# mxy-kit/poisson-ellipse-openmp-mpi-cuda

Hardware: AMD Instinct MI355X
Metric: pcg_iters_per_sec_8192x8192 (higher is better)
Workload: dtype fp64

## Files before the change

csrc/hip/fused3.hip:

```cpp
#include <cstdlib>

#include "peer_sum.hpp"
#include "sstep.hpp"

#pragma clang fp contract(fast)

namespace pe {
namespace dev {

namespace {

constexpr int H3 = 6;
constexpr int FSW3 = kFSW3;
constexpr int HL3 = kHL3, HR3 = 64 - kFSW3 - kHL3;
static_assert(HL3 >= H3 && HR3 >= H3, "three-step strip: 64 loaded columns (one per lane), >= H3 halo lanes per side");
#ifndef PE_S3_XD
#define PE_S3_XD 3
#endif
#ifndef PE_S3_WD
#define PE_S3_WD 3
#endif
#ifndef PE_S3_NTX
#define PE_S3_NTX 0
#endif
constexpr int kS3XD = PE_S3_XD, kS3WD = PE_S3_WD;
static_assert(6 % kS3XD == 0 && 6 % kS3WD == 0, "register ring periods must divide the 6-step group");
constexpr int NS = kNS3;
constexpr int kRing3 = 7;
using WaveTV3 = WaveTV1<kRing3>;

struct Coef3 {
  double zc[3], a[3], b[3], cw[3];
};

struct Scal3 {
  bool first;
  long long K;
  int m;
  int brk;
  bool bad;
  Coef3 c;
  double g[3];
};

__device__ __forceinline__ double mform(const double (&xz)[3], const double (&xp)[3], const double (&mzz)[6],
                                        const double (&mzp)[6], const double (&mpp)[6], int sh) {
  double s = 0.0;
#pragma unroll
  for (int a = 0; a < 3; ++a)
#pragma unroll
    for (int b = 0; b < 3; ++b) {
      const int n = a + b + sh;
      s += xz[a] * (xz[b] * mzz[n] + 2.0 * xp[b] * mzp[n]) + xp[a] * xp[b] * mpp[n];
    }
  return s;
}

struct St3 {
  long long iter, brk3, k0;
  int done, late3, wpar, started, bad3;
  double gprev;
  double n2[2][3];
  double sc[12];
  double R[16];
};
__device__ __forceinline__ St3 st3_load(const DevState* st, int par) {
  St3 S;
  S.done = st->done;
  S.iter = st->iter;
  S.late3 = st->late3;
  S.wpar = st->wpar;
  S.started = st->started;
  S.bad3 = st->bad3;
  S.brk3 = st->brk3;
  S.k0 = st->k0;
  S.gprev = st->gprev;
#pragma unroll
  for (int i = 0; i < 3; ++i) {
    S.n2[0][i] = st->fs2[0][16 + i];
    S.n2[1][i] = st->fs2[1][16 + i];
  }
#pragma unroll
  for (int i = 0; i < 12; ++i) S.sc[i] = st->sc3[i];
  const double* R = st->fs2[par ^ 1];
#pragma unroll
  for (int i = 0; i < 16; ++i) S.R[i] = R[i];
  return S;
}

__device__ __forceinline__ Scal3 sweep3_scalars(const KParams& k, const St3& st, int par) {
  Scal3 c;
  c.first = st.started == 0;
  c.K = st.iter;
  c.m = 0;
  c.brk = 0;
  c.bad = false;
#pragma unroll
  for (int i = 0; i < 3; ++i) {
    c.c.zc[i] = 0.0;
    c.c.a[i] = 0.0;
    c.c.b[i] = 1.0;
    c.c.cw[i] = 0.0;
    c.g[i] = 0.0;
  }
  if (c.first) return c;
  const double hh = k.h1 * k.h2;
// ... 119 lines not shown
  p.n = m0;
#pragma unroll
  for (int i = 0; i < 3; ++i)
    if (i < m0) {
      p.d[i] = late_diff(k, st, i);
      p.a[i] = st.sc[3 + i];
      p.b[i] = st.sc[6 + i];
      p.g[i] = st.sc[9 + i];
    }
}
__device__ __forceinline__ void pend3_record(const KParams& k, DevState* st, const Pend3& p) {
#pragma unroll
  for (int i = 0; i < 3; ++i)
    if (i < p.n) {
      hist_put(k, p.K0 + i + 1, p.d[i]);
      if (i + 1 == p.n) {
        st->last_diff = p.d[i];
        st->alpha = p.a[i];
        st->beta = p.b[i];
        st->rz_cur = p.g[i];
      }
    }
}

__device__ __forceinline__ void sweep3_finalize(const KParams& k, DevState* st, int par, const Scal3& c,
                                                const double (&t)[NS], const Pend3& pend) {
  if (!c.first) pend3_record(k, st, pend);
#pragma unroll
  for (int n = 0; n < NS; ++n) st->fs2[par][n] = t[n];
  if (!c.first && k.fault_iter > c.K && k.fault_iter <= c.K + c.m) st->fs2[par][1] = __builtin_nan("");
  if (!c.first && k.fault_zero > c.K && k.fault_zero <= c.K + c.m)
    st->fs2[par][1] = st->fs2[par][6] = st->fs2[par][11] = 0.0;
  st->wpend = 0;
  st->wpar = par;
  if (c.first) {
    st->started = 1;
    return;
  }
#pragma unroll
  for (int i = 0; i < 3; ++i) {
    st->sc3[i] = c.c.zc[i];
    st->sc3[3 + i] = c.c.a[i];
    st->sc3[6 + i] = c.c.b[i];
    st->sc3[9 + i] = c.g[i];
    if (i + 1 == c.m) {
      st->alpha = c.c.a[i];
      st->beta = c.c.b[i];
      st->rz_cur = c.g[i];
      st->gprev = c.g[i];
    }
  }
  st->iter = c.K + c.m;
  st->late3 = c.m;
  st->brk3 = c.brk ? c.K + c.brk : 0;
  st->bad3 = c.bad ? 1 : 0;
}

enum { kMixed = 0, kBand = 1, kUniform = 2 };

struct M3Ctx {
  const double* Xm;
  double* Ym;
  double* Wm;
  const double* hrd;
  int64_t pitch, poff, wp;
  int J, c0, ib, ie, t0, tmax, nx, par;
  unsigned off;
  bool lv0, o0, fix;
  bool scol;
  double lf0;
  double ih1, ih2, dcl;
  int rlo, rhi;
  double zc1, zc2, zc3, a1, a2, a3, b1, b2, b3, w1, w2, w3;
};

struct M3Rings {
  double RQ[kS3XD], PQ[kS3XD], WQ[kS3WD];
  double P1[3], RI[2], R1[2], P2[3], R2[2], P3[3], Z[3], S[2], U[3], V[3], UU[3], VV[3];
  bool pushed;
};

typedef __attribute__((address_space(1))) char gchar3;
typedef __attribute__((address_space(1))) double gdouble3;
struct M3Ptr {
  const gchar3* xi;
  gchar3* yo;
  gchar3* wo;
  unsigned pb, wb;
  unsigned roff, poffb, wloff;
};

struct Pre3 {
  int2 e;
  int4 rc4;
  bool staged;
};

template <bool STEADY>
__device__ __forceinline__ URow urow(const M3Ctx& c, int q) {
  URow r{c.ih1, c.ih2, c.dcl};
  if constexpr (!STEADY) {
    if (!(q >= c.rlo && q <= c.rhi)) r.d = 0.0;
  }
  return r;
}

template <bool PUSH>
__device__ __forceinline__ double ldx3(const KParams& k, const M3Ctx& c, int t, unsigned o) {
  if constexpr (PUSH) {
    if ((t < 1 && k.has[LEFT]) || (t > c.nx && k.has[RIGHT])) {
      const double* h = c.hrd + int64_t(t < 1 ? t + H3 - 1 : t - c.nx + H3 - 1) * c.pitch + o;
      return __hip_atomic_load(h, __ATOMIC_RELAXED, __HIP_MEMORY_SCOPE_SYSTEM);
    }
  }
#if PE_S3_NTX
  return __builtin_nontemporal_load(c.Xm + int64_t(t) * c.pitch + o);
#else
  return c.Xm[int64_t(t) * c.pitch + o];
#endif
}

__device__ __forceinline__ double ldxb3(const gchar3* base, unsigned& off) {
  asm("" : "+v"(off));
#if PE_S3_NTX
  return __builtin_nontemporal_load(reinterpret_cast<const gdouble3*>(base + off));
#else
  return *reinterpret_cast<const gdouble3*>(base + off);
#endif
}
__device__ __forceinline__ double ldntb3(const gchar3* base, unsigned& off) {
  asm("" : "+v"(off));
  return __builtin_nontemporal_load(reinterpret_cast<const gdouble3*>(base + off));
}
__device__ __forceinline__ void stntb3(gchar3* base, unsigned& off, double v) {
  asm("" : "+v"(off));
  __builtin_nontemporal_store(v, reinterpret_cast<gdouble3*>(base + off));
}

__device__ __forceinline__ double ldnt1(const double* p) { return __builtin_nontemporal_load(p); }
__device__ __forceinline__ void stnt1(double* p, double v) { __builtin_nontemporal_store(v, p); }

__device__ __forceinline__ void push_row3(const KParams& k, const M3Ctx& c, M3Rings& x, int q, double r3, double p3) {
  auto put = [&](double* base, int slot) {
    double* d = base + int64_t(slot) * c.pitch + c.off;
    if (c.o0) {
      __hip_atomic_store(d, r3, __ATOMIC_RELAXED, __HIP_MEMORY_SCOPE_SYSTEM);
      __hip_atomic_store(d + c.poff, p3, __ATOMIC_RELAXED, __HIP_MEMORY_SCOPE_SYSTEM);
    }
    x.pushed = true;
  };
  if (q <= H3 && k.hpush_lo[c.par] != nullptr) put(k.hpush_lo[c.par], q - 1);
  if (q >= c.nx - H3 + 1 && k.hpush_hi[c.par] != nullptr) put(k.hpush_hi[c.par], q - (c.nx - H3 + 1));
}

template <int KIND, bool PUSH, bool EDGE, bool STEADY, int JJ>
__device__ __forceinline__ void step3(const KParams& k, const M3Ctx& c, M3Rings& x, M3Ptr& rp, const RowCtx& rx,
                                      WaveTV3& tvw, double (&sv)[NS], int n, int bs) {
  constexpr bool BAND = KIND == kBand, UNI = KIND == kUniform;
  constexpr int XD = kS3XD, WD = kS3WD;
  const double zc1 = c.zc1, zc2 = c.zc2, zc3 = c.zc3, w1 = c.w1, w2 = c.w2, w3 = c.w3;
  constexpr int m0 = JJ % 3, m1 = (JJ + 2) % 3, m2 = (JJ + 1) % 3;
  constexpr int e0 = JJ & 1, e1 = (JJ + 1) & 1;
  constexpr int xs = JJ % XD, ws = JJ % WD;
  const int t = c.t0 + n;
  const int c0 = c.c0;
  auto inr = [&](int q) { return STEADY ? !c.fix : (q >= c.ib && q <= c.ie); };
  auto own = [&](int q) { return STEADY || (q >= c.ib && q <= c.ie); };
  auto put = [&](int n, double v) {
    if constexpr (UNI) sv[n] += v;
    else sv[n] += c.scol ? v : 0.0;
  };
  auto interior = [&](int q) { return q >= c.rlo && q <= c.rhi; };
  auto live = [&](int d) { return STEADY || n >= 2 * d; };
  int bsl[7];
#pragma unroll
  for (int d = 0; d < 7; ++d) bsl[d] = bs >= d ? bs - d : bs - d + kRing3;
  auto zmask = [&](int q, double v, double d) -> double {
    if constexpr (UNI) {
      return EDGE ? (v * d) * c.lf0 : v * d;
    } else {
      return (interior(q) && c.lv0) ? v * d : 0.0;
    }
  };
  auto op = [&](int q, int sl, int sln, double um, double u0, double un, double& d) {
    if constexpr (UNI) {
      const URow r = urow<STEADY>(c, q);
      d = r.d;
      return lapu(r, um, u0, un);
    } else {
      return apply_row1<BAND>(k, rx, tvw, q, c0, sl, sln, um, u0, un, d);
    }
  };
  auto pnext = [&](double zc, double z, double b, double p, bool zfused) -> double {
    if constexpr (UNI) return zfused ? __builtin_fma(zc, z, b * p) : __builtin_fma(b, p, zc * z);
    else return zc * z + b * p;
  };
  constexpr bool kAzf = STEADY && (PUSH ? JJ >= 3 : (!EDGE && JJ >= 4));
  const double rin = x.RQ[xs], pin = x.PQ[xs], wrow = x.WQ[ws];
  if constexpr (STEADY) {
    const int tn = t + XD;
    if (PUSH && ((tn < 1 && k.has[LEFT]) || (tn > c.nx && k.has[RIGHT]))) {
      x.RQ[xs] = ldx3<PUSH>(k, c, tn, c.off);
      x.PQ[xs] = ldx3<PUSH>(k, c, tn, unsigned(c.poff) + c.off);
    } else {
      x.RQ[xs] = ldxb3(rp.xi, rp.roff);
      x.PQ[xs] = ldxb3(rp.xi, rp.poffb);
    }
    x.WQ[ws] = c.o0 ? ldntb3(rp.wo, rp.wloff) : 0.0;
  } else {
    const int tn = min(t + XD, c.tmax);
    x.RQ[xs] = ldx3<PUSH>(k, c, tn, c.off);
    x.PQ[xs] = ldx3<PUSH>(k, c, tn, unsigned(c.poff) + c.off);
    const int wr = min(max(t - 2 + WD, c.ib), c.ie);
    x.WQ[ws] = c.o0 ? ldnt1(c.Wm + int64_t(wr) * c.wp + c.off) : 0.0;
  }
  {
    double d;
    if constexpr (UNI) d = urow<STEADY>(c, t).d;
    else d = BAND ? enter_band1(k, rx, tvw, t, c0, bsl[0]) : dinv_plain1(k, rx, t, c0);
    const double z = zmask(t, rin, d);
    x.P1[m0] = pnext(zc1, z, c.b1, pin, kAzf);
    x.RI[e0] = rin;
  }
  if (STEADY) __builtin_amdgcn_sched_barrier(0);
  if (live(1)) {
    const int q = t - 1;
    double d;
    const double s1 = op(q, bsl[1], bsl[0], x.P1[m2], x.P1[m1], x.P1[m0], d);
    const double r1 = x.RI[e1] - c.a1 * s1;
    const double z = zmask(q, r1, d);
    const double p1 = x.P1[m1];
    x.R1[e1] = r1;
    x.P2[m1] = pnext(zc2, z, c.b2, p1, false);
    if (inr(q)) put(16, p1 * p1);
  }
  if (STEADY) __builtin_amdgcn_sched_barrier(0);
  if (live(2)) {
    const int q = t - 2;
    double d;
    const double s2 = op(q, bsl[2], bsl[1], x.P2[m0], x.P2[m2], x.P2[m1], d);
    const double r2 = x.R1[e0] - c.a2 * s2;
    const double z = zmask(q, r2, d);
    const double p2 = x.P2[m2];
    x.R2[e0] = r2;
    const double p3 = pnext(zc3, z, c.b3, p2, false);
    x.P3[m2] = p3;
    if (own(q) && c.o0) {
      const double wn = wrow + w1 * x.P1[m2] + w2 * p2 + w3 * p3;
      if constexpr (STEADY) stntb3(rp.wo, rp.roff, wn);
      else stnt1(c.Wm + int64_t(q) * c.wp + c.off, wn);
    }
    if (inr(q)) put(17, p2 * p2);
  }
  if (STEADY) __builtin_amdgcn_sched_barrier(0);
  if (live(3)) {
    const int q = t - 3;
    double d;
    const double s3 = op(q, bsl[3], bsl[2], x.P3[m1], x.P3[m0], x.P3[m2], d);
    const double r3 = x.R2[e1] - c.a3 * s3;
    const double z = zmask(q, r3, d);
    x.Z[m0] = z;
    x.S[e1] = s3;
    const double p3 = x.P3[m0];
    if (own(q) && !c.fix) {
      if (c.o0) {
        if constexpr (STEADY) {
          stntb3(rp.yo, rp.roff, r3);
          stntb3(rp.yo, rp.poffb, p3);
        } else {
          double* yr = c.Ym + int64_t(q) * c.pitch + c.off;
          stnt1(yr, r3);
          stnt1(yr + c.poff, p3);
        }
      }
      if constexpr (PUSH) push_row3(k, c, x, q, r3, p3);
    }
    if (inr(q)) {
      put(0, r3 * z);
      put(6, z * s3);
      put(11, p3 * s3);
      put(18, p3 * p3);
    }
  }
  if (STEADY) __builtin_amdgcn_sched_barrier(0);
  if (live(4)) {
    const int q = t - 4;
    double d;
    const double qv = op(q, bsl[4], bsl[3], x.Z[m2], x.Z[m1], x.Z[m0], d);
    const double sr = x.S[e0];
    const double u = zmask(q, qv, d);
    const double v = zmask(q, sr, d);
    x.U[m1] = u;
    x.V[m1] = v;
    if (inr(q)) {
      put(1, x.Z[m1] * qv);
      put(2, qv * u);
      put(7, qv * v);
      put(12, sr * v);
    }
  }
  if (STEADY) __builtin_amdgcn_sched_barrier(0);
  if (live(5)) {
    const int q = t - 5;
    double d, d2;
    const double au = op(q, bsl[5], bsl[4], x.U[m0], x.U[m2], x.U[m1], d);
    const double av = op(q, bsl[5], bsl[4], x.V[m0], x.V[m2], x.V[m1], d2);
    const double uu = zmask(q, au, d);
    const double vv = zmask(q, av, d);
    x.UU[m2] = uu;
    x.VV[m2] = vv;
    if (inr(q)) {
      const double u = x.U[m2], v = x.V[m2];
      put(3, u * au);
      put(8, u * av);
      put(13, v * av);
      put(4, au * uu);
      put(9, au * vv);
      put(14, av * vv);
    }
  }
  if (STEADY) __builtin_amdgcn_sched_barrier(0);
  {
    const int q = t - 6;
    if (inr(q)) {
      double d;
      const double auu = op(q, bsl[6], bsl[5], x.UU[m1], x.UU[m0], x.UU[m2], d);
      const double avv = op(q, bsl[6], bsl[5], x.VV[m1], x.VV[m0], x.VV[m2], d);
      const double uu = x.UU[m0], vv = x.VV[m0];
      put(5, uu * auu);
      put(10, uu * avv);
      put(15, vv * avv);
    }
  }
  if constexpr (STEADY) {
    rp.xi += rp.pb;
    rp.yo += rp.pb;
    rp.wo += rp.wb;
    asm("" : "+s"(rp.xi), "+s"(rp.yo), "+s"(rp.wo));
  }
}

template <int KIND, bool PUSH, bool EDGE, bool STEADY>
__device__ __forceinline__ void group3(const KParams& k, const M3Ctx& c, M3Rings& x, M3Ptr& rp, const RowCtx& rx,
                                       WaveTV3& tvw, double (&sv)[NS], int n0, int nsteps, int& bs) {
  auto adv = [&]() { bs = bs == kRing3 - 1 ? 0 : bs + 1; };
#define PE_STEP3(JJ)                                                              \
  if (STEADY || n0 + JJ < nsteps) {                                               \
    step3<KIND, PUSH, EDGE, STEADY, JJ>(k, c, x, rp, rx, tvw, sv, n0 + JJ, bs);   \
    adv();                                                                        \
    if (STEADY) __builtin_amdgcn_sched_barrier(0);                                \
  }
  PE_STEP3(0)
  PE_STEP3(1)
  PE_STEP3(2)
  PE_STEP3(3)
  PE_STEP3(4)
  PE_STEP3(5)
#undef PE_STEP3
}

__device__ __forceinline__ unsigned long long rtc3() {
  unsigned long long t;
  asm volatile("s_memrealtime %0\n\ts_waitcnt lgkmcnt(0)" : "=s"(t)::"memory");
  return t;
}

__device__ __forceinline__ void prio_turn(const KParams& k) {
  if (k.prio > 0) {
    const unsigned long long t = rtc3();
    const bool young = int(blockIdx.x) >= k.ncu;
    if ((((t >> k.prio) & 1ull) != 0) != young) __builtin_amdgcn_s_setprio(1);
    else __builtin_amdgcn_s_setprio(0);
  }
}

template <int KIND, bool PUSH, bool EDGE, bool SST = false>
__device__ __forceinline__ void march3(const KParams& k, const Coef3& cf, bool fix, int par, int s, int ib, int ie,
                                       WaveTV3& tvw, double (&sv)[NS], unsigned long long* sst, const Pre3& pre,
                                       bool use_pre) {
  const int lane = threadIdx.x & 63;
  const int ny = int(k.ny);
  M3Ctx c;
  c.pitch = k.pitch;
  c.poff = k.poff;
  c.wp = k.wpitch;
  c.Xm = k.x[par ^ 1] - (HL3 - 1);
  c.Ym = k.x[par] - (HL3 - 1);
  c.Wm = k.w - (HL3 - 1);
  c.J = -(HL3 - 1) + s * FSW3;
  c.c0 = c.J + lane;
  c.off = unsigned(c.c0 + HL3 - 1);
  const int64_t g0 = k.gj0 + c.c0;
  c.lv0 = c.c0 <= ny + H3 && g0 >= 1 && g0 <= k.N - 1;
  c.lf0 = c.lv0 ? 1.0 : 0.0;
  c.o0 = lane >= HL3 && lane < 64 - HR3 && c.c0 >= 1 && c.c0 <= ny;
  c.scol = c.c0 <= ny;
  c.fix = fix;
  c.ib = ib;
  c.ie = ie;
  c.t0 = ib - H3;
  c.tmax = ie + H3;
  c.nx = int(k.nx);
  c.par = par;
  c.hrd = PUSH ? k.hrecv + int64_t(par ^ 1) * 2 * H3 * k.pitch : nullptr;
  c.rlo = int(max<int64_t>(1 - k.gi0, -(1 << 30)));
  c.rhi = int(min<int64_t>(k.M - 1 - k.gi0, 1 << 30));
  c.zc1 = cf.zc[0];
  c.zc2 = cf.zc[1];
  c.zc3 = cf.zc[2];
  c.a1 = cf.a[0];
  c.a2 = cf.a[1];
  c.a3 = cf.a[2];
  c.b1 = cf.b[0];
  c.b2 = cf.b[1];
  c.b3 = cf.b[2];
  c.w1 = cf.cw[0];
  c.w2 = cf.cw[1];
  c.w3 = cf.cw[2];
  asm("" : "+v"(c.w1), "+v"(c.w2), "+v"(c.w3));

  RowCtx rx;
  auto load_seg = [&](int base) { load_rows<KIND == kBand, WaveTV3, 64>(k, rx, tvw, base, ie + H3 + 1, c.J); };
  if (KIND == kBand) load_strip_tables1(k, tvw, c.c0);
  if (use_pre) load_rows<KIND == kBand, WaveTV3, 64>(k, rx, tvw, c.t0, ie + H3 + 1, c.J, &pre.rc4);
  else load_seg(c.t0);
  if constexpr (KIND == kUniform) {
    const bool in = rx.allin & 1ull;
    c.ih1 = in ? k.ih1sq : uni(k.inv_eps * k.ih1sq);
    c.ih2 = in ? k.ih2sq : uni(k.inv_eps * k.ih2sq);
    c.dcl = in ? k.dinv_in : k.dinv_out;
  } else {
    c.ih1 = c.ih2 = c.dcl = 0.0;
  }

  M3Rings x;
  x.pushed = false;
  constexpr int XD = kS3XD, WD = kS3WD;
  static_assert(WD <= 6, "the first WD w rows are all row ib (t0 - 2 + q < ib)");
  if (use_pre && pre.staged && KIND != kBand) {
    asm volatile("s_waitcnt vmcnt(0)" ::: "memory");
    const double* L = &tvw.a0r[0][0];
#pragma unroll
    for (int q = 0; q < XD; ++q) {
      x.RQ[q] = L[q * 128 + lane];
      x.PQ[q] = L[q * 128 + 64 + lane];
    }
    const double w0 = L[XD * 128 + lane];
#pragma unroll
    for (int q = 0; q < WD; ++q) x.WQ[q] = c.o0 ? w0 : 0.0;
  } else {
#pragma unroll
    for (int q = 0; q < XD; ++q) {
      const int t = min(c.t0 + q, c.tmax);
      x.RQ[q] = ldx3<PUSH>(k, c, t, c.off);
      x.PQ[q] = ldx3<PUSH>(k, c, t, unsigned(c.poff) + c.off);
    }
#pragma unroll
    for (int q = 0; q < WD; ++q)
      x.WQ[q] = c.o0 ? ldnt1(c.Wm + int64_t(min(max(c.t0 - 2 + q, ib), ie)) * c.wp + c.off) : 0.0;
  }
#pragma unroll
  for (int q = 0; q < 3; ++q) x.P1[q] = x.P2[q] = x.P3[q] = x.Z[q] = x.U[q] = x.V[q] = x.UU[q] = x.VV[q] = 0.0;
#pragma unroll
  for (int q = 0; q < 2; ++q) x.RI[q] = x.R1[q] = x.R2[q] = x.S[q] = 0.0;

  const int nsteps = ie + H3 - c.t0 + 1;
  const int rows = ie - ib + 1;
  int bs = 0;
  int sg = 3;
  if constexpr (SST) {
    if (sst && lane == 0) sst[2] = rtc3();
  }
  auto sstamp = [&]() {
    if constexpr (SST) {
      if (sst && lane == 0 && sg < 28) sst[sg] = rtc3();
      ++sg;
    }
    prio_turn(k);
  };
  auto reload = [&](int n0) {
    if (KIND != kUniform && c.t0 + n0 + 6 - rx.segbase > 63) load_seg(c.t0 + n0 - H3);
  };
  M3Ptr rp;
  rp.pb = unsigned(c.pitch) * 8u;
  rp.wb = unsigned(c.wp) * 8u;
  rp.roff = c.off * 8u;
  rp.poffb = (unsigned(c.poff) + c.off) * 8u;
  rp.wloff = rp.roff + unsigned(WD) * rp.wb;
  rp.xi = nullptr;
  rp.yo = rp.wo = nullptr;
  int n0 = 0;
  const int nsteady_end = KIND == kUniform ? rows + 4 - 5 : -1;
  for (; n0 < nsteps && !(n0 >= 12 && n0 <= nsteady_end); n0 += 6) {
    reload(n0);
    group3<KIND, PUSH, EDGE, false>(k, c, x, rp, rx, tvw, sv, n0, nsteps, bs);
    sstamp();
  }
  if constexpr (KIND == kUniform) {
    rp.xi = (const gchar3*)(c.Xm + int64_t(c.t0 + n0 + XD) * c.pitch);
    rp.yo = (gchar3*)(c.Ym + int64_t(c.t0 + n0 - 3) * c.pitch);
    rp.wo = (gchar3*)(c.Wm + int64_t(c.t0 + n0 - 2) * c.wp);
    for (; n0 <= nsteady_end; n0 += 6) {
      reload(n0);
      group3<KIND, PUSH, EDGE, true>(k, c, x, rp, rx, tvw, sv, n0, nsteps, bs);
      sstamp();
    }
    for (; n0 < nsteps; n0 += 6) {
      reload(n0);
      group3<KIND, PUSH, EDGE, false>(k, c, x, rp, rx, tvw, sv, n0, nsteps, bs);
      sstamp();
    }
  }
  if constexpr (PUSH) {
    if (x.pushed) asm volatile("s_waitcnt vmcnt(0)" ::: "memory");
  }
}

__device__ __forceinline__ void pre_load3(const KParams& k, int gwave, Pre3& pr) {
  pr.e = make_int2(0, 0);
  if (!(gwave < k.lwaves && gwave < k.nslots)) return;
  pr.e = cload_i2(k.ilist + gwave);
  const int rows = pr.e.y >> 20;
  if (rows == 0) return;
  const int ib = pr.e.x & kRowMask3;
  const int ie = min(ib + rows - 1, int(k.nx));
  pr.rc4 = rowcls_entry(k, ib - H3, ie + H3 + 1);
}

template <bool PUSH>
__device__ __forceinline__ void stage_first3(const KParams& k, int par, WaveTV3& tv, Pre3& pr) {
  pr.staged = false;
  const int rows = pr.e.y >> 20;
  if (rows == 0 || !k.stage || (pr.e.x & kBandBit)) return;
  const int sx = pr.e.y & 0xFFFFF, ib = pr.e.x & kRowMask3;
  const int t0 = ib - H3;
  if (PUSH && (t0 < 1 || t0 + kS3XD - 1 > int(k.nx))) return;
  typedef __attribute__((address_space(3))) void* lds_ptr;
  typedef __attribute__((address_space(1))) const void* g_ptr;
  const int lane = threadIdx.x & 63;
  const double* Xm = k.x[par ^ 1] - (HL3 - 1) + sx * FSW3;
  const double* Wm = k.w - (HL3 - 1) + sx * FSW3;
  static_assert((kS3XD * 128 + 64) * sizeof(double) <= sizeof(tv.a0r) + sizeof(tv.b0r), "staged rows fit the face ring");
  double* L = &tv.a0r[0][0];
#pragma unroll
  for (int q = 0; q < kS3XD; ++q) {
    const char* rr = reinterpret_cast<const char*>(Xm + int64_t(t0 + q) * k.pitch);
    const char* pp = reinterpret_cast<const char*>(Xm + int64_t(t0 + q) * k.pitch + k.poff);
#pragma unroll
    for (int h = 0; h < 2; ++h) {
      __builtin_amdgcn_global_load_lds((g_ptr)(rr + 256 * h + 4 * lane), (lds_ptr)(L + q * 128 + 32 * h), 4, 0, 0);
      __builtin_amdgcn_global_load_lds((g_ptr)(pp + 256 * h + 4 * lane), (lds_ptr)(L + q * 128 + 64 + 32 * h), 4, 0, 0);
    }
  }
  const char* wr = reinterpret_cast<const char*>(Wm + int64_t(ib) * k.wpitch);
#pragma unroll
  for (int h = 0; h < 2; ++h)
    __builtin_amdgcn_global_load_lds((g_ptr)(wr + 256 * h + 4 * lane), (lds_ptr)(L + kS3XD * 128 + 32 * h), 4, 0, 0);
  pr.staged = true;
}

__device__ __forceinline__ Coef3 uni3(const Coef3& c) {
  Coef3 u;
#pragma unroll
  for (int i = 0; i < 3; ++i) {
    u.zc[i] = uni(c.zc[i]);
    u.a[i] = uni(c.a[i]);
    u.b[i] = uni(c.b[i]);
    u.cw[i] = uni(c.cw[i]);
  }
  return u;
}

enum { kPlain = 0, kStamp = 1, kReplay = 2, kSignal = 3 };

template <bool PUSH, int MODE>
__device__ __forceinline__ void walk3(const KParams& k, const Coef3& cf, bool fix, int par, WaveTV3& tv, int wid,
                                      double (&acc)[NS], const Pre3& pre, bool have_pre) {
  constexpr bool STAMP = MODE == kStamp;
  const int W = k.lwaves;
  const int gwave = int(blockIdx.x) * kWPB + wid;
  const bool l0 = (threadIdx.x & 63) == 0;
  if constexpr (STAMP) {
    if (l0) k.stamps[4 * int64_t(k.nslots) + 2 * gwave] = rtc3();
  }
  const int pend = gwave < W ? k.nslots : 0;
  unsigned long long* sst = STAMP ? k.stamps2 + 32 * int64_t(gwave) : nullptr;
  bool p1 = have_pre && !fix;
  bool ring_zeroed = false;
  for (int pos = gwave; pos < pend; pos += W) {
    const int2 e = p1 ? pre.e : cload_i2(k.ilist + pos);
    const int rows = e.y >> 20;
    if (rows == 0) {
      p1 = false;
      continue;
    }
    const int s = e.y & 0xFFFFF, ib = e.x & kRowMask3;
    const int ie = min(ib + rows - 1, int(k.nx));
    const unsigned long long t_item = STAMP ? rtc3() : 0ull;
    if constexpr (STAMP) {
      if (sst && l0) sst[0] = t_item;
    }
    if (e.x & kBandBit) {
      if (!ring_zeroed) {
        if (have_pre && pre.staged) asm volatile("s_waitcnt vmcnt(0)" ::: "memory");
        const int ln = threadIdx.x & 63;
        for (int i = ln; i < kRing3 * 64; i += 64) (&tv.a0r[0][0])[i] = 0.0;
        for (int i = ln; i < kRing3 * 66; i += 64) (&tv.b0r[0][0])[i] = 0.0;
        for (int i = ln; i < kRing3 * 64; i += 64) (&tv.d0r[0][0])[i] = 0.0;
        ring_zeroed = true;
      }
      march3<kBand, PUSH, true, STAMP>(k, cf, fix, par, s, ib, ie, tv, acc, sst, pre, p1);
    } else if (e.x & kUniBit) {
      const int c0 = -(HL3 - 1) + s * FSW3 + int(threadIdx.x & 63);
      const int64_t g0 = k.gj0 + c0;
      const bool lv = c0 <= int(k.ny) + H3 && g0 >= 1 && g0 <= k.N - 1;
      if (__ballot(lv) == ~0ull) march3<kUniform, PUSH, false, STAMP>(k, cf, fix, par, s, ib, ie, tv, acc, sst, pre, p1);
      else march3<kUniform, PUSH, true, STAMP>(k, cf, fix, par, s, ib, ie, tv, acc, sst, pre, p1);
    } else {
      march3<kMixed, PUSH, true, STAMP>(k, cf, fix, par, s, ib, ie, tv, acc, sst, pre, p1);
    }
    p1 = false;
    if constexpr (STAMP) {
      if (sst && l0) sst[31] = rtc3();
      sst = nullptr;
    }
    if constexpr (MODE == kSignal) {
      if (pos < k.lnb[0]) {
        asm volatile("s_waitcnt vmcnt(0)" ::: "memory");
        if (l0) __hip_atomic_fetch_add(&k.st->sig, 1ull, __ATOMIC_RELAXED, __HIP_MEMORY_SCOPE_AGENT);
      }
    }
    if constexpr (STAMP) {
      if (l0) {
        const unsigned long long kind = (e.x & kBandBit) ? 1ull : (e.x & kUniBit) ? 2ull : 0ull;
        unsigned long long* d = k.stamps + 4 * int64_t(pos);
        d[0] = t_item;
        d[1] = rtc3();
        d[2] = (unsigned long long)gwave | ((unsigned long long)s << 32);
        d[3] = (unsigned long long)ib | ((unsigned long long)(ie - ib + 1) << 32) | (kind << 48);
      }
    }
  }
  if constexpr (STAMP) {
    if (l0) {
      k.stamps[4 * int64_t(k.nslots) + 2 * gwave + 1] = rtc3();
      k.stamps2[32 * int64_t(gwave) + 29] = __builtin_amdgcn_s_memtime();
    }
  }
}

template <bool PUSH, int MODE = kPlain>
__global__ __launch_bounds__(TJ) __attribute__((amdgpu_waves_per_eu(2))) void kS3(KParams k, int par) {
  DevState* st = k.st;
  const St3 S = st3_load(st, par);
  const int done = S.done;
  __shared__ double sm[4 * NS];
  __shared__ int sflag;
  __shared__ WaveTV3 tvs[kWPB];
  __shared__ Pend3 pend;
  __shared__ Scal3 scl;
  const int lane = int(threadIdx.x & 63);
  const int wid = __builtin_amdgcn_readfirstlane(int(threadIdx.x >> 6));
  constexpr bool replay = MODE == kReplay;
  if constexpr (MODE == kStamp) {
    const unsigned long long t_in = rtc3();
    if (lane == 0) {
      k.stamps2[32 * (int64_t(blockIdx.x) * kWPB + wid) + 1] = t_in;
      const unsigned hw = __builtin_amdgcn_s_getreg(4 | (31 << 11)), xcc = __builtin_amdgcn_s_getreg(20 | (31 << 11));
      k.stamps2[32 * (int64_t(blockIdx.x) * kWPB + wid) + 30] = hw | (static_cast<unsigned long long>(xcc) << 32);
      k.stamps2[32 * (int64_t(blockIdx.x) * kWPB + wid) + 28] = __builtin_amdgcn_s_memtime();
      if (blockIdx.x == 0 && wid == 0) k.stamps2[-8] = k.stamps2[-6];
    }
  }
  if (done && !replay) return;
  Pre3 pre;
  const bool use_pre = !replay && k.pre_load;
  if (use_pre) {
    pre_load3(k, int(blockIdx.x) * kWPB + wid, pre);
    stage_first3<PUSH>(k, par, tvs[wid], pre);
  } else {
    pre.staged = false;
  }
  auto finish = [&](int upto, long long iter, int status, int fixj = 0) {
    if (arrive_last_wave(&st->ticket[4], gridDim.x * kWPB) && lane == 0) {
      sweep3_stop(k, st, upto, iter, status, fixj);
      __hip_atomic_store(&st->ticket[4], 0u, __ATOMIC_RELAXED, __HIP_MEMORY_SCOPE_AGENT);
    }
  };
  double acc[NS];
#pragma unroll
  for (int n = 0; n < NS; ++n) acc[n] = 0.0;
  const int m0 = S.late3;
  const long long K = S.iter, K0 = K - m0;
  auto pstamp = [&](int slot, double dep) {
// ... 145 lines not shown
```

csrc/hip/placement.cpp:

```cpp
#include <hip/hip_runtime_api.h>

#include <algorithm>
#include <chrono>
#include <cmath>
#include <cstdio>
#include <cstring>
#include <map>
#include <limits>
#include <mutex>
#include <queue>
#include <string>
#include <vector>

#include <rocprofiler-sdk-roctx/roctx.h>

#include "../hip/kernels.hpp"
#include "env_knobs.hpp"
#include "pe/device.hpp"
#include "solver_internal.hpp"

namespace pe {

namespace detail {
void* field_try_alloc(size_t bytes) {
  void* p = nullptr;
  if (hipMalloc(&p, bytes) != hipSuccess) {
    (void)hipGetLastError();
    return nullptr;
  }
  return p;
}

void* field_alloc(size_t bytes) {
  void* p = field_try_alloc(bytes);
  if (!p) PE_HIP_CHECK(hipErrorOutOfMemory);
  return p;
}

void field_free(void* p) {
  if (p) (void)hipFree(p);
}
}

using detail::clk;
using detail::field_free;
using detail::field_try_alloc;
using detail::Range;
using detail::secs;
using dev::KParams;

void DeviceSolver::choose_placement() {
  const double t_all = placement_s_;
  const auto t0 = clk::now();
  const bool fast = placement_search(false);
  if (comm_->size() > 1) {
    double v[1] = {(!placement_ms_.empty() && !fast) ? 1.0 : 0.0};
    comm_->host_max(v, 1, stream_);
    if (v[0] > 0.0 && !placement_ms_.empty() && !fast) placement_search(true);
    double m[1] = {placement_ms_.empty() ? 0.0 : double(placement_ms_[size_t(placement_best_)])};
    comm_->host_max(m, 1, stream_);
    placement_job_ms_ = m[0];
  } else if (!placement_ms_.empty()) {
    placement_job_ms_ = placement_ms_[size_t(placement_best_)];
  }
  placement_s_ = t_all + secs(t0, clk::now());
}

bool DeviceSolver::placement_search(bool retry) {
  Range range("pe.placement_search");
  double search_s = 0;
  struct Clock {
    double& out;
    clk::time_point t0 = clk::now();
    ~Clock() { out = secs(t0, clk::now()); }
  } clock{search_s};
  const double pts = double(blk_.nx) * double(blk_.ny);
  int tries = pts >= 24.0e6 ? 12 : 1;
  if (retry) tries = std::max(1, tries / 2 + 1);
  if (const std::optional<int> e = read_env_knobs().placement_tries) tries = std::max(1, *e);
  const double skip_gb = 8.0;
  const bool mid_large = pts < 50.0e6;
  const double fast_tbs = steps_ >= 3 ? (mid_large ? 4.0 : 4.6) : sstep_ ? 4.7 : 4.9, max_s = 0.3;
  if (tries <= 1) return true;
  {
    const double frac = 0.4;
    size_t free_b = 0, total_b = 0;
    if (hipMemGetInfo(&free_b, &total_b) == hipSuccess) {
      const double per_try = skip_gb * double(1ull << 30) + double(sizeof(double) * (2 * geo_.xsize + geo_.wsize));
      tries = std::min<int>(tries, std::max(1, int(frac * double(free_b) / per_try)));
    }
  }
  if (tries <= 1) return true;
  struct Cand {
    double *x0, *x1, *w;
    float ms;
  };
  std::vector<Cand> c;
  std::vector<void*> spacers;
  c.push_back(Cand{fields_, xalt_, walt_, 0.f});
  const size_t n_first = placement_ms_.size();
  if (retry && skip_gb > 0) {
    const double gb = double(n_first) * (skip_gb + double(sizeof(double) * (2 * geo_.xsize + geo_.wsize)) / double(1ull << 30));
    void* sp = nullptr;
    if (hipMalloc(&sp, size_t(gb * double(1ull << 30))) == hipSuccess) spacers.push_back(sp);
    else (void)hipGetLastError();
  }
  bool fast = false;
  for (int t = 0; t < tries; ++t) {
    if (t > 0) {
      void* sp = nullptr;
      if (skip_gb > 0 && hipMalloc(&sp, size_t(skip_gb * double(1ull << 30))) != hipSuccess) break;
      if (sp) spacers.push_back(sp);
      void* a = field_try_alloc(sizeof(double) * geo_.xsize);
      if (!a) break;
      void* b = field_try_alloc(sizeof(double) * geo_.xsize);
      if (!b) {
        field_free(a);
        break;
      }
      void* w = field_try_alloc(sizeof(double) * geo_.wsize);
      if (!w) {
        field_free(a);
        field_free(b);
        break;
      }
      c.push_back(Cand{static_cast<double*>(a), static_cast<double*>(b), static_cast<double*>(w), 0.f});
    }
    set_fused_fields(c[t].x0, c[t].x1, c[t].w);
    enqueue_init();
    dev::launch_S(*kp_, 1, stream_);
    for (int i = 0; i < 2; ++i) dev::launch_S(*kp_, i & 1, stream_);
    PE_HIP_CHECK(hipEventRecord(t0_, stream_));
    for (int i = 0; i < 6; ++i) dev::launch_S(*kp_, i & 1, stream_);
    PE_HIP_CHECK(hipEventRecord(t1_, stream_));
    PE_HIP_CHECK(hipEventSynchronize(t1_));
    PE_HIP_CHECK(hipEventElapsedTime(&c[t].ms, t0_, t1_));
    const double bps = sstep_ ? 48.0 : 40.0;
    const double tbs = bps * pts / (double(c[t].ms) / 6.0 * 1e-3) / 1e12;
    if (tbs >= fast_tbs) {
      fast = true;
      break;
    }
    if (secs(clock.t0, clk::now()) > max_s) break;
  }
  (void)hipGetLastError();
  size_t best = 0;
  for (size_t i = 1; i < c.size(); ++i)
    if (c[i].ms < c[best].ms) best = i;
  for (size_t i = 0; i < c.size(); ++i)
    if (i != best) {
      field_free(c[i].x0);
      field_free(c[i].x1);
      field_free(c[i].w);
    }
  for (void* sp : spacers) PE_HIP_CHECK(hipFree(sp));
  set_fused_fields(c[best].x0, c[best].x1, c[best].w);
  if (!retry) placement_ms_.clear();
  placement_best_ = int(placement_ms_.size() + best);
  for (const Cand& x : c) placement_ms_.push_back(x.ms / 6.0f);
  return fast || mid_large || (sstep_ ? 48.0 : 40.0) * pts / (double(c[best].ms) / 6.0 * 1e-3) / 1e12 >= fast_tbs;
}

}
```

csrc/hip/sstep.hpp:

```cpp
#pragma once

#include "kcommon.hpp"

#pragma clang fp contract(fast)

namespace pe {
namespace dev {
namespace {

__device__ __forceinline__ double2 dd(double a, double b) { return make_double2(a, b); }
__device__ __forceinline__ int2 cload_i2(const int2* p) {
  const long long v = cload(reinterpret_cast<const long long*>(p));
  return make_int2(int(v), int(v >> 32));
}

__device__ __forceinline__ double uni(double x) {
  const long long v = __double_as_longlong(x);
  const unsigned lo = unsigned(__builtin_amdgcn_readfirstlane(int(unsigned(v))));
  const unsigned hi = unsigned(__builtin_amdgcn_readfirstlane(int(v >> 32)));
  return __longlong_as_double((long long)((unsigned long long)hi << 32 | lo));
}

__device__ __forceinline__ double vreg(double x) {
  asm volatile("; vreg %0" : "+v"(x));
// ... 100 lines not shown
  double2 d, a0, b0;
  if (gen) {
    const int l = (q - rx.segbase) & 63;
    const int4 r4 = tv.rc[l];
    const RowCls rc{r4.x, r4.y, r4.z, r4.w};
    const CT ct{tv.half[l], tv.half[l + 1], tv.sB[l], tv.eB[l]};
    const CS x0 = cset_rc(k, rc, ct, c0, TV{tv.sA[jl], tv.eA[jl], tv.hB[jl], tv.hB[jl + 1]});
    const CS x1 = cset_rc(k, rc, ct, c0 + 1, TV{tv.sA[jl + 1], tv.eA[jl + 1], tv.hB[jl + 1], tv.hB[jl + 2]});
    d = dd(x0.d, x1.d);
    a0 = dd(x0.a0, x1.a0);
    b0 = dd(x0.b0, x1.b0);
  } else {
    const double f0 = in0 ? 1.0 : k.inv_eps, f1 = in1 ? 1.0 : k.inv_eps;
    d = dd(in0 ? k.dinv_in : k.dinv_out, in1 ? k.dinv_in : k.dinv_out);
    a0 = dd(f0, f1);
    b0 = a0;
  }
  *reinterpret_cast<double2*>(&tv.a0r[sl][jl]) = a0;
  *reinterpret_cast<double2*>(&tv.b0r[sl][jl]) = b0;
  __builtin_amdgcn_fence(__ATOMIC_RELEASE, "wavefront");
  __builtin_amdgcn_wave_barrier();
  __builtin_amdgcn_fence(__ATOMIC_ACQUIRE, "wavefront");
  return d;
}

template <bool BAND, class WT>
__device__ __forceinline__ double2 apply_row(const KParams& k, const RowCtx& rx, const WT& tv, int q, int c0, int jl,
                                             int sl, int sln, const double2& um, const double2& u0, const double2& un,
                                             double2& d) {
  const double ul = dpp_shr1(u0.y), ur = dpp_shl1(u0.x);
  bool in0, in1, gen;
  row_in(rx, q, c0, in0, in1, gen);
  if (BAND && gen) {
    const double2 a0 = *reinterpret_cast<const double2*>(&tv.a0r[sl][jl]);
    const double2 a1 = *reinterpret_cast<const double2*>(&tv.a0r[sln][jl]);
    const double2 b0 = *reinterpret_cast<const double2*>(&tv.b0r[sl][jl]);
    const double b2 = tv.b0r[sl][jl + 2];
    const CS x0{a0.x, a1.x, b0.x, b0.y, dinv_faces(k, a0.x, a1.x, b0.x, b0.y)};
    const CS x1{a0.y, a1.y, b0.y, b2, dinv_faces(k, a0.y, a1.y, b0.y, b2)};
    d = dd(x0.d, x1.d);
    return dd(stencil<false>(k, x0, um.x, u0.x, un.x, ul, u0.y), stencil<false>(k, x1, um.y, u0.y, un.y, u0.x, ur));
  }
  d = dd(in0 ? k.dinv_in : k.dinv_out, in1 ? k.dinv_in : k.dinv_out);
  return dd(lap(k, in0 ? 1.0 : k.inv_eps, um.x, u0.x, un.x, ul, u0.y),
            lap(k, in1 ? 1.0 : k.inv_eps, um.y, u0.y, un.y, u0.x, ur));
}

__device__ __forceinline__ double2 dinv_plain(const KParams& k, const RowCtx& rx, int q, int c0) {
  bool in0, in1, gen;
  row_in(rx, q, c0, in0, in1, gen);
  return dd(in0 ? k.dinv_in : k.dinv_out, in1 ? k.dinv_in : k.dinv_out);
}

__device__ __forceinline__ double dot2(const double2& a, const double2& b) { return a.x * b.x + a.y * b.y; }

template <int RING>
struct WaveTV1 {
  double sA[64], eA[64], hB[66];
  int4 rc[64];
  double half[65], sB[64], eB[64];
  double a0r[RING][64];
  double b0r[RING][66];
  double d0r[RING][64];
};

template <class WT>
__device__ __forceinline__ void load_strip_tables1(const KParams& k, WT& tvw, int c0) {
  const int lane = threadIdx.x & 63;
  const double* tb = k.rowT + (c0 + 1) * 4;
  tvw.sA[lane] = tb[0];
  tvw.eA[lane] = tb[1];
  tvw.hB[lane] = tb[2];
  if (lane == 63) tvw.hB[64] = tb[6];
}

__device__ __forceinline__ void row_in1(const RowCtx& rx, int q, int c0, bool& in0, bool& gen) {
  const int l = (q - rx.segbase) & 63;
  const int lo = __builtin_amdgcn_readlane(rx.rcv.x, l), hi = __builtin_amdgcn_readlane(rx.rcv.y, l);
  in0 = c0 >= lo && c0 <= hi;
  gen = (rx.genmask >> l) & 1ull;
}

template <class WT>
__device__ __forceinline__ double enter_band1(const KParams& k, const RowCtx& rx, WT& tv, int q, int c0, int sl) {
  const int lane = threadIdx.x & 63;
  bool in0, gen;
  row_in1(rx, q, c0, in0, gen);
  double d, a0, b0;
  if (gen) {
    const int l = (q - rx.segbase) & 63;
    const int4 r4 = tv.rc[l];
    const RowCls rc{r4.x, r4.y, r4.z, r4.w};
    const CT ct{tv.half[l], tv.half[l + 1], tv.sB[l], tv.eB[l]};
    const CS x0 = cset_rc(k, rc, ct, c0, TV{tv.sA[lane], tv.eA[lane], tv.hB[lane], tv.hB[lane + 1]});
    d = x0.d;
    a0 = x0.a0;
    b0 = x0.b0;
  } else {
    d = in0 ? k.dinv_in : k.dinv_out;
    a0 = b0 = in0 ? 1.0 : k.inv_eps;
  }
  tv.a0r[sl][lane] = a0;
  tv.b0r[sl][lane] = b0;
  tv.d0r[sl][lane] = d;
  __builtin_amdgcn_fence(__ATOMIC_RELEASE, "wavefront");
  __builtin_amdgcn_wave_barrier();
  __builtin_amdgcn_fence(__ATOMIC_ACQUIRE, "wavefront");
  return d;
}

template <bool BAND, class WT>
__device__ __forceinline__ double apply_row1(const KParams& k, const RowCtx& rx, const WT& tv, int q, int c0, int sl,
                                             int sln, double um, double u0, double un, double& d) {
  const int lane = threadIdx.x & 63;
  const double ul = dpp_shr1(u0), ur = dpp_shl1(u0);
  bool in0, gen;
  row_in1(rx, q, c0, in0, gen);
  if (BAND && gen) {
    const double a0 = tv.a0r[sl][lane], a1 = tv.a0r[sln][lane];
    const double b0 = tv.b0r[sl][lane], b1 = tv.b0r[sl][lane + 1];
    const CS x0{a0, a1, b0, b1, k.dring ? tv.d0r[sl][lane] : dinv_faces(k, a0, a1, b0, b1)};
    d = x0.d;
    return stencil<false>(k, x0, um, u0, un, ul, ur);
  }
  d = in0 ? k.dinv_in : k.dinv_out;
  return lap(k, in0 ? 1.0 : k.inv_eps, um, u0, un, ul, ur);
}

struct URow {
  double ih1, ih2, d;
};

__device__ __forceinline__ double lapu(const URow& r, double um, double u0, double un) {
  const double e = u0 - dpp_shr1(u0);
  return ((u0 - um) - (un - u0)) * r.ih1 + (e - dpp_shl1(e)) * r.ih2;
}

__device__ __forceinline__ double dinv_plain1(const KParams& k, const RowCtx& rx, int q, int c0) {
  bool in0, gen;
  row_in1(rx, q, c0, in0, gen);
  return in0 ? k.dinv_in : k.dinv_out;
}

}
}
}
```

Before: 4464.

## Use buffer-resource stores/loads for Y and W rows with sentinel offsets for masked lanes

In the uniform three-step kernel, the Y and W row accesses are switched from flat global pointers to raw buffer loads and stores through a wave-uniform buffer resource. Lanes that should not write or read get an out-of-range sentinel offset, so the buffer's range check drops them instead of a per-lane branch. Row advancement is now done through a scalar offset, and an optional waitcnt drain is added before the steady loop. The placement search also raises its early-exit throughput threshold for large grids and warms up the first candidate longer, which changes which memory placement is chosen.

```diff
diff --git a/csrc/hip/fused3.hip b/csrc/hip/fused3.hip
--- a/csrc/hip/fused3.hip
+++ b/csrc/hip/fused3.hip
@@ -19,6 +19,9 @@
 #endif
 #ifndef PE_S3_WD
 #define PE_S3_WD 3
+#endif
+#ifndef PE_S3_DRAIN
+#define PE_S3_DRAIN 1
 #endif
 #ifndef PE_S3_NTX
 #define PE_S3_NTX 0
@@ -307,13 +310,38 @@
 
 typedef __attribute__((address_space(1))) char gchar3;
 typedef __attribute__((address_space(1))) double gdouble3;
+typedef __amdgpu_buffer_rsrc_t rsrc3;
+typedef unsigned v2u3 __attribute__((ext_vector_type(2)));
+constexpr unsigned kBufRecs = 0x40000000u;
+constexpr unsigned kBufSent = 0x80000000u;
+constexpr int kBufNT = 2;
 struct M3Ptr {
   const gchar3* xi;
-  gchar3* yo;
-  gchar3* wo;
+  rsrc3 yr, wr;
+  unsigned ys, ws;
   unsigned pb, wb;
-  unsigned roff, poffb, wloff;
+  unsigned roff, poffb;
+  unsigned wsoff, wloff, yroff, ypoff;
 };
+
+__device__ __forceinline__ rsrc3 rsrc_rows3(const void* row) {
+  const unsigned long long a = reinterpret_cast<unsigned long long>(row);
+  const unsigned lo = unsigned(__builtin_amdgcn_readfirstlane(int(unsigned(a))));
+  const unsigned hi = unsigned(__builtin_amdgcn_readfirstlane(int(unsigned(a >> 32))));
+  void* p = reinterpret_cast<void*>((unsigned long long)hi << 32 | lo);
+  return __builtin_amdgcn_make_buffer_rsrc(p, 0, int(kBufRecs), 0x00020000);
+}
+__device__ __forceinline__ double ldntq3(rsrc3 r, unsigned off, unsigned soff) {
+  const v2u3 v = __builtin_amdgcn_raw_buffer_load_b64(r, int(off), int(soff), kBufNT);
+  return __longlong_as_double((long long)((unsigned long long)v.y << 32 | v.x));
+}
+__device__ __forceinline__ void stntq3(rsrc3 r, unsigned off, unsigned soff, double x) {
+  const unsigned long long b = (unsigned long long)__double_as_longlong(x);
+  v2u3 v;
+  v.x = unsigned(b);
+  v.y = unsigned(b >> 32);
+  __builtin_amdgcn_raw_buffer_store_b64(v, r, int(off), int(soff), kBufNT);
+}
 
 struct Pre3 {
   int2 e;
@@ -352,14 +380,6 @@
 #else
   return *reinterpret_cast<const gdouble3*>(base + off);
 #endif
-}
-__device__ __forceinline__ double ldntb3(const gchar3* base, unsigned& off) {
-  asm("" : "+v"(off));
-  return __builtin_nontemporal_load(reinterpret_cast<const gdouble3*>(base + off));
-}
-__device__ __forceinline__ void stntb3(gchar3* base, unsigned& off, double v) {
-  asm("" : "+v"(off));
-  __builtin_nontemporal_store(v, reinterpret_cast<gdouble3*>(base + off));
 }
 
 __device__ __forceinline__ double ldnt1(const double* p) { return __builtin_nontemporal_load(p); }
@@ -431,13 +451,14 @@
       x.RQ[xs] = ldxb3(rp.xi, rp.roff);
       x.PQ[xs] = ldxb3(rp.xi, rp.poffb);
     }
-    x.WQ[ws] = c.o0 ? ldntb3(rp.wo, rp.wloff) : 0.0;
+    x.WQ[ws] = ldntq3(rp.wr, rp.wloff, rp.ws);
   } else {
     const int tn = min(t + XD, c.tmax);
     x.RQ[xs] = ldx3<PUSH>(k, c, tn, c.off);
     x.PQ[xs] = ldx3<PUSH>(k, c, tn, unsigned(c.poff) + c.off);
     const int wr = min(max(t - 2 + WD, c.ib), c.ie);
-    x.WQ[ws] = c.o0 ? ldnt1(c.Wm + int64_t(wr) * c.wp + c.off) : 0.0;
+    if constexpr (UNI) x.WQ[ws] = ldntq3(rp.wr, rp.wsoff, unsigned(wr - c.ib) * rp.wb);
+    else x.WQ[ws] = c.o0 ? ldnt1(c.Wm + int64_t(wr) * c.wp + c.off) : 0.0;
   }
   {
     double d;
@@ -470,10 +491,14 @@
     x.R2[e0] = r2;
     const double p3 = pnext(zc3, z, c.b3, p2, false);
     x.P3[m2] = p3;
-    if (own(q) && c.o0) {
+    if constexpr (UNI) {
+      if (own(q)) {
+        const double wn = wrow + w1 * x.P1[m2] + w2 * p2 + w3 * p3;
+        stntq3(rp.wr, rp.wsoff, STEADY ? rp.ws : unsigned(q - c.ib) * rp.wb, wn);
+      }
+    } else if (own(q) && c.o0) {
       const double wn = wrow + w1 * x.P1[m2] + w2 * p2 + w3 * p3;
-      if constexpr (STEADY) stntb3(rp.wo, rp.roff, wn);
-      else stnt1(c.Wm + int64_t(q) * c.wp + c.off, wn);
+      stnt1(c.Wm + int64_t(q) * c.wp + c.off, wn);
     }
     if (inr(q)) put(17, p2 * p2);
   }
@@ -487,16 +512,20 @@
     x.Z[m0] = z;
     x.S[e1] = s3;
     const double p3 = x.P3[m0];
-    if (own(q) && !c.fix) {
+    if constexpr (UNI) {
+      if (own(q)) {
+        const unsigned so = STEADY ? rp.ys : unsigned(q - c.ib) * rp.pb;
+        stntq3(rp.yr, rp.yroff, so, r3);
+        stntq3(rp.yr, rp.ypoff, so, p3);
+        if constexpr (PUSH) {
+          if (!c.fix) push_row3(k, c, x, q, r3, p3);
+        }
+      }
+    } else if (own(q) && !c.fix) {
       if (c.o0) {
-        if constexpr (STEADY) {
-          stntb3(rp.yo, rp.roff, r3);
-          stntb3(rp.yo, rp.poffb, p3);
-        } else {
-          double* yr = c.Ym + int64_t(q) * c.pitch + c.off;
-          stnt1(yr, r3);
-          stnt1(yr + c.poff, p3);
-        }
+        double* yr = c.Ym + int64_t(q) * c.pitch + c.off;
+        stnt1(yr, r3);
+        stnt1(yr + c.poff, p3);
       }
       if constexpr (PUSH) push_row3(k, c, x, q, r3, p3);
     }
@@ -559,9 +588,9 @@
   }
   if constexpr (STEADY) {
     rp.xi += rp.pb;
-    rp.yo += rp.pb;
-    rp.wo += rp.wb;
-    asm("" : "+s"(rp.xi), "+s"(rp.yo), "+s"(rp.wo));
+    rp.ys += rp.pb;
+    rp.ws += rp.wb;
+    asm("" : "+s"(rp.xi), "+s"(rp.ys), "+s"(rp.ws));
   }
 }
 
@@ -711,9 +740,18 @@
   rp.wb = unsigned(c.wp) * 8u;
   rp.roff = c.off * 8u;
   rp.poffb = (unsigned(c.poff) + c.off) * 8u;
-  rp.wloff = rp.roff + unsigned(WD) * rp.wb;
   rp.xi = nullptr;
-  rp.yo = rp.wo = nullptr;
+  rp.ys = rp.ws = 0u;
+  if constexpr (KIND == kUniform) {
+    rp.yr = rsrc_rows3(c.Ym + int64_t(ib) * c.pitch);
+    rp.wr = rsrc_rows3(c.Wm + int64_t(ib) * c.wp);
+    const bool oy = c.o0 && !fix;
+    rp.wsoff = c.o0 ? rp.roff : kBufSent;
+    rp.wloff = c.o0 ? rp.roff + unsigned(WD) * rp.wb : kBufSent;
+    rp.yroff = oy ? rp.roff : kBufSent;
+    rp.ypoff = oy ? rp.poffb : kBufSent;
+    asm("" : "+v"(rp.wsoff), "+v"(rp.wloff), "+v"(rp.yroff), "+v"(rp.ypoff));
+  }
   int n0 = 0;
   const int nsteady_end = KIND == kUniform ? rows + 4 - 5 : -1;
   for (; n0 < nsteps && !(n0 >= 12 && n0 <= nsteady_end); n0 += 6) {
@@ -723,8 +761,11 @@
   }
   if constexpr (KIND == kUniform) {
     rp.xi = (const gchar3*)(c.Xm + int64_t(c.t0 + n0 + XD) * c.pitch);
-    rp.yo = (gchar3*)(c.Ym + int64_t(c.t0 + n0 - 3) * c.pitch);
-    rp.wo = (gchar3*)(c.Wm + int64_t(c.t0 + n0 - 2) * c.wp);
+    rp.ys = unsigned(c.t0 + n0 - 3 - ib) * rp.pb;
+    rp.ws = unsigned(c.t0 + n0 - 2 - ib) * rp.wb;
+#if PE_S3_DRAIN
+    if (n0 <= nsteady_end) __builtin_amdgcn_s_waitcnt(0x0F70);
+#endif
     for (; n0 <= nsteady_end; n0 += 6) {
       reload(n0);
       group3<KIND, PUSH, EDGE, true>(k, c, x, rp, rx, tvw, sv, n0, nsteps, bs);
diff --git a/csrc/hip/placement.cpp b/csrc/hip/placement.cpp
--- a/csrc/hip/placement.cpp
+++ b/csrc/hip/placement.cpp
@@ -80,7 +80,7 @@
   if (const std::optional<int> e = read_env_knobs().placement_tries) tries = std::max(1, *e);
   const double skip_gb = 8.0;
   const bool mid_large = pts < 50.0e6;
-  const double fast_tbs = steps_ >= 3 ? (mid_large ? 4.0 : 4.6) : sstep_ ? 4.7 : 4.9, max_s = 0.3;
+  const double fast_tbs = steps_ >= 3 ? (mid_large ? 4.0 : 4.9) : sstep_ ? 4.7 : 4.9, max_s = 0.3;
   if (tries <= 1) return true;
   {
     const double frac = 0.4;
@@ -106,6 +106,7 @@
     else (void)hipGetLastError();
   }
   bool fast = false;
+  constexpr int kFirstTryWarm = 20;
   for (int t = 0; t < tries; ++t) {
     if (t > 0) {
       void* sp = nullptr;
@@ -129,7 +130,7 @@
     set_fused_fields(c[t].x0, c[t].x1, c[t].w);
     enqueue_init();
     dev::launch_S(*kp_, 1, stream_);
-    for (int i = 0; i < 2; ++i) dev::launch_S(*kp_, i & 1, stream_);
+    for (int i = 0; i < (t == 0 && steps_ >= 3 ? kFirstTryWarm : 2); ++i) dev::launch_S(*kp_, i & 1, stream_);
     PE_HIP_CHECK(hipEventRecord(t0_, stream_));
     for (int i = 0; i < 6; ++i) dev::launch_S(*kp_, i & 1, stream_);
     PE_HIP_CHECK(hipEventRecord(t1_, stream_));
```

Result: slower. 4413 (-1.1%).

## Extend steady-state path to band strips with register-carried slot and gen ring

Applied to the files above, without the earlier changes.

Band strips now use the unrolled steady-state march that was previously reserved for uniform strips. The per-step row classification (readlane of row bounds and the gen mask) is replaced by a shifted bitmask of gen flags and a compile-time-rotated slot table. Non-gen rows read their coefficient and diagonal from the LDS ring instead of recomputing them from row bounds. It also turns the non-uniform pnext into an explicit fma, adds an optional wave-priority knob for band strips that defaults to off, and pins some uniform scalars in SGPRs. The cost is more LDS reads per step and extra register pressure from the carried slot array.

```diff
diff --git a/csrc/hip/fused3.hip b/csrc/hip/fused3.hip
--- a/csrc/hip/fused3.hip
+++ b/csrc/hip/fused3.hip
@@ -22,6 +22,9 @@
 #endif
 #ifndef PE_S3_NTX
 #define PE_S3_NTX 0
+#endif
+#ifndef PE_S3_BPRIO
+#define PE_S3_BPRIO 0
 #endif
 constexpr int kS3XD = PE_S3_XD, kS3WD = PE_S3_WD;
 static_assert(6 % kS3XD == 0 && 6 % kS3WD == 0, "register ring periods must divide the 6-step group");
@@ -321,6 +324,11 @@
   bool staged;
 };
 
+struct M3Band {
+  int sl[kRing3];
+  unsigned gen;
+};
+
 template <bool STEADY>
 __device__ __forceinline__ URow urow(const M3Ctx& c, int q) {
   URow r{c.ih1, c.ih2, c.dcl};
@@ -380,7 +388,7 @@
 
 template <int KIND, bool PUSH, bool EDGE, bool STEADY, int JJ>
 __device__ __forceinline__ void step3(const KParams& k, const M3Ctx& c, M3Rings& x, M3Ptr& rp, const RowCtx& rx,
-                                      WaveTV3& tvw, double (&sv)[NS], int n, int bs) {
+                                      WaveTV3& tvw, double (&sv)[NS], int n, M3Band& bd) {
   constexpr bool BAND = KIND == kBand, UNI = KIND == kUniform;
   constexpr int XD = kS3XD, WD = kS3WD;
   const double zc1 = c.zc1, zc2 = c.zc2, zc3 = c.zc3, w1 = c.w1, w2 = c.w2, w3 = c.w3;
@@ -399,12 +407,13 @@
   auto live = [&](int d) { return STEADY || n >= 2 * d; };
   int bsl[7];
 #pragma unroll
-  for (int d = 0; d < 7; ++d) bsl[d] = bs >= d ? bs - d : bs - d + kRing3;
+  for (int d = 0; d < 7; ++d) bsl[d] = bd.sl[(d - JJ + kRing3) % kRing3];
+  auto gen = [&](int d) { return ((bd.gen >> d) & 1u) != 0; };
   auto zmask = [&](int q, double v, double d) -> double {
     if constexpr (UNI) {
       return EDGE ? (v * d) * c.lf0 : v * d;
     } else {
-      return (interior(q) && c.lv0) ? v * d : 0.0;
+      return ((STEADY || interior(q)) && c.lv0) ? v * d : 0.0;
     }
   };
   auto op = [&](int q, int sl, int sln, double um, double u0, double un, double& d) {
@@ -412,13 +421,15 @@
       const URow r = urow<STEADY>(c, q);
       d = r.d;
       return lapu(r, um, u0, un);
+    } else if constexpr (BAND) {
+      return apply_ring1(k, tvw, gen(t - q), sl, sln, um, u0, un, d);
     } else {
-      return apply_row1<BAND>(k, rx, tvw, q, c0, sl, sln, um, u0, un, d);
+      return apply_row1<false>(k, rx, tvw, q, c0, sl, sln, um, u0, un, d);
     }
   };
   auto pnext = [&](double zc, double z, double b, double p, bool zfused) -> double {
     if constexpr (UNI) return zfused ? __builtin_fma(zc, z, b * p) : __builtin_fma(b, p, zc * z);
-    else return zc * z + b * p;
+    else return __builtin_fma(b, p, zc * z);
   };
   constexpr bool kAzf = STEADY && (PUSH ? JJ >= 3 : (!EDGE && JJ >= 4));
   const double rin = x.RQ[xs], pin = x.PQ[xs], wrow = x.WQ[ws];
@@ -442,7 +453,11 @@
   {
     double d;
     if constexpr (UNI) d = urow<STEADY>(c, t).d;
-    else d = BAND ? enter_band1(k, rx, tvw, t, c0, bsl[0]) : dinv_plain1(k, rx, t, c0);
+    else if constexpr (BAND) {
+      bool g;
+      d = enter_band1(k, rx, tvw, t, c0, bsl[0], g);
+      bd.gen = (bd.gen << 1) | (g ? 1u : 0u);
+    } else d = dinv_plain1(k, rx, t, c0);
     const double z = zmask(t, rin, d);
     x.P1[m0] = pnext(zc1, z, c.b1, pin, kAzf);
     x.RI[e0] = rin;
@@ -567,12 +582,10 @@
 
 template <int KIND, bool PUSH, bool EDGE, bool STEADY>
 __device__ __forceinline__ void group3(const KParams& k, const M3Ctx& c, M3Rings& x, M3Ptr& rp, const RowCtx& rx,
-                                       WaveTV3& tvw, double (&sv)[NS], int n0, int nsteps, int& bs) {
-  auto adv = [&]() { bs = bs == kRing3 - 1 ? 0 : bs + 1; };
+                                       WaveTV3& tvw, double (&sv)[NS], int n0, int nsteps, M3Band& bd) {
 #define PE_STEP3(JJ)                                                              \
   if (STEADY || n0 + JJ < nsteps) {                                               \
-    step3<KIND, PUSH, EDGE, STEADY, JJ>(k, c, x, rp, rx, tvw, sv, n0 + JJ, bs);   \
-    adv();                                                                        \
+    step3<KIND, PUSH, EDGE, STEADY, JJ>(k, c, x, rp, rx, tvw, sv, n0 + JJ, bd);   \
     if (STEADY) __builtin_amdgcn_sched_barrier(0);                                \
   }
   PE_STEP3(0)
@@ -582,6 +595,12 @@
   PE_STEP3(4)
   PE_STEP3(5)
 #undef PE_STEP3
+  if constexpr (KIND == kBand) {
+    const int s0 = bd.sl[0];
+#pragma unroll
+    for (int i = 0; i + 1 < kRing3; ++i) bd.sl[i] = bd.sl[i + 1];
+    bd.sl[kRing3 - 1] = s0;
+  }
 }
 
 __device__ __forceinline__ unsigned long long rtc3() {
@@ -691,7 +710,10 @@
 
   const int nsteps = ie + H3 - c.t0 + 1;
   const int rows = ie - ib + 1;
-  int bs = 0;
+  M3Band bd;
+  bd.gen = 0;
+#pragma unroll
+  for (int i = 0; i < kRing3; ++i) bd.sl[i] = i == 0 ? 0 : kRing3 - i;
   int sg = 3;
   if constexpr (SST) {
     if (sst && lane == 0) sst[2] = rtc3();
@@ -715,24 +737,30 @@
   rp.xi = nullptr;
   rp.yo = rp.wo = nullptr;
   int n0 = 0;
-  const int nsteady_end = KIND == kUniform ? rows + 4 - 5 : -1;
+  constexpr bool kSteady = KIND == kUniform || KIND == kBand;
+  const int nsteady_end = kSteady ? rows + 4 - 5 : -1;
   for (; n0 < nsteps && !(n0 >= 12 && n0 <= nsteady_end); n0 += 6) {
     reload(n0);
-    group3<KIND, PUSH, EDGE, false>(k, c, x, rp, rx, tvw, sv, n0, nsteps, bs);
+    group3<KIND, PUSH, EDGE, false>(k, c, x, rp, rx, tvw, sv, n0, nsteps, bd);
     sstamp();
   }
-  if constexpr (KIND == kUniform) {
+  if constexpr (kSteady) {
     rp.xi = (const gchar3*)(c.Xm + int64_t(c.t0 + n0 + XD) * c.pitch);
     rp.yo = (gchar3*)(c.Ym + int64_t(c.t0 + n0 - 3) * c.pitch);
     rp.wo = (gchar3*)(c.Wm + int64_t(c.t0 + n0 - 2) * c.wp);
+    M3Ctx cs = c;
+    if constexpr (KIND == kUniform) {
+      asm("" : "+s"(cs.a1), "+s"(cs.a2), "+s"(cs.a3), "+s"(rp.wb), "+s"(rp.pb));
+      if constexpr (PUSH || SST) asm("" : "+s"(cs.zc1), "+s"(cs.zc2), "+s"(cs.zc3), "+s"(cs.b1), "+s"(cs.b2), "+s"(cs.b3));
+    }
     for (; n0 <= nsteady_end; n0 += 6) {
       reload(n0);
-      group3<KIND, PUSH, EDGE, true>(k, c, x, rp, rx, tvw, sv, n0, nsteps, bs);
+      group3<KIND, PUSH, EDGE, true>(k, cs, x, rp, rx, tvw, sv, n0, nsteps, bd);
       sstamp();
     }
     for (; n0 < nsteps; n0 += 6) {
       reload(n0);
-      group3<KIND, PUSH, EDGE, false>(k, c, x, rp, rx, tvw, sv, n0, nsteps, bs);
+      group3<KIND, PUSH, EDGE, false>(k, c, x, rp, rx, tvw, sv, n0, nsteps, bd);
       sstamp();
     }
   }
@@ -834,7 +862,9 @@
         for (int i = ln; i < kRing3 * 64; i += 64) (&tv.d0r[0][0])[i] = 0.0;
         ring_zeroed = true;
       }
+      if (PE_S3_BPRIO) __builtin_amdgcn_s_setprio(1);
       march3<kBand, PUSH, true, STAMP>(k, cf, fix, par, s, ib, ie, tv, acc, sst, pre, p1);
+      if (PE_S3_BPRIO) __builtin_amdgcn_s_setprio(0);
     } else if (e.x & kUniBit) {
       const int c0 = -(HL3 - 1) + s * FSW3 + int(threadIdx.x & 63);
       const int64_t g0 = k.gj0 + c0;
diff --git a/csrc/hip/sstep.hpp b/csrc/hip/sstep.hpp
--- a/csrc/hip/sstep.hpp
+++ b/csrc/hip/sstep.hpp
@@ -206,9 +206,10 @@
 }
 
 template <class WT>
-__device__ __forceinline__ double enter_band1(const KParams& k, const RowCtx& rx, WT& tv, int q, int c0, int sl) {
-  const int lane = threadIdx.x & 63;
-  bool in0, gen;
+__device__ __forceinline__ double enter_band1(const KParams& k, const RowCtx& rx, WT& tv, int q, int c0, int sl,
+                                              bool& gen) {
+  const int lane = threadIdx.x & 63;
+  bool in0;
   row_in1(rx, q, c0, in0, gen);
   double d, a0, b0;
   if (gen) {
@@ -251,6 +252,22 @@
   return lap(k, in0 ? 1.0 : k.inv_eps, um, u0, un, ul, ur);
 }
 
+template <class WT>
+__device__ __forceinline__ double apply_ring1(const KParams& k, const WT& tv, bool gen, int sl, int sln, double um,
+                                              double u0, double un, double& d) {
+  const int lane = threadIdx.x & 63;
+  const double ul = dpp_shr1(u0), ur = dpp_shl1(u0);
+  if (gen) {
+    const double a0 = tv.a0r[sl][lane], a1 = tv.a0r[sln][lane];
+    const double b0 = tv.b0r[sl][lane], b1 = tv.b0r[sl][lane + 1];
+    const CS x0{a0, a1, b0, b1, k.dring ? tv.d0r[sl][lane] : dinv_faces(k, a0, a1, b0, b1)};
+    d = x0.d;
+    return stencil<false>(k, x0, um, u0, un, ul, ur);
+  }
+  d = tv.d0r[sl][lane];
+  return lap(k, tv.a0r[sl][lane], um, u0, un, ul, ur);
+}
+
 struct URow {
   double ih1, ih2, d;
 };
```

After: 4454 before, 4605 after (median of 6 runs). +3.4%, better.
